# ZhangHH233/Retinal_OCT_Image_Segmentation_via_Deep_Learning

Hardware: AMD Instinct MI355X
Metric: B-scans/sec (train fwd+bwd) at batch 32, 512x1024 (higher is better)
Workload: dtype bf16; 1 GPU; SOTAS/Layers_Segment UNet(1,8,init_features=32) train step, 512x1024, batch 32/GPU (BASELINE configs[1]); global_batch=32, parallelism=dp1, hip_graph=False

## Files before the change

include/oct_hip.h:

```cpp
#ifndef OCT_HIP_H
#define OCT_HIP_H

#include <stddef.h>
#include <stdint.h>

#ifdef __cplusplus
extern "C" {
#endif

#define OCT_VERSION 220

#define OCT_DT_BF16 0
#define OCT_DT_F32 1

#define OCT_OK 0
#define OCT_IMG_SHIFT_ALL 2
#define OCT_E_INVALID (-22)
#define OCT_E_LAUNCH (-5)
#define OCT_E_NODEVICE (-19)

#define OCT_XF_NONE 0
#define OCT_XF_AFFINE_RELU 1
#define OCT_XF_AFFINE 2

// ... 19 lines not shown
int oct_device_count(void);

typedef struct OctConvDesc {
  int dtype;
  int n, h, w;
  int c0, c1;
  int cout;
  int taps;
  int xform0, xform1;
  int in_mode, out_mode;
  int split;
  int want_stats;
  int kh, kw;
  int depth;
  int out_img_mul, out_img_add;
} OctConvDesc;

typedef struct OctConvArgs {
  const void* x0; const void* x1;
  const float* scale0; const float* shift0;
  const float* scale1; const float* shift1;
  const void* wpacked;
  const float* bias;
  void* y0; void* y1;
  float* stat_partials;
} OctConvArgs;

int oct_conv_stat_blocks(const OctConvDesc* d);
size_t oct_packed_weight_elems(int rows, int taps, int kch);
int oct_pack_weights(int mode, int dtype, const float* w, void* wpacked, int cout, int cin, void* stream);
int oct_pack_weights_kk(int mode, int dtype, const float* w, void* wpacked, int cout, int cin, int kh, int kw,
                        void* stream);
int oct_pack_weights3d(int mode, int dtype, const float* w, void* wpacked, int cout, int cin, int kdi, void* stream);
#define OCT_PACK_BATCH_MAX 96
typedef struct OctPackJob {
  int mode, cout, cin, reserved;
  const float* w;
  void* wpacked;
} OctPackJob;
int oct_pack_weights_batch(int dtype, int count, const OctPackJob* jobs, void* stream);
int oct_conv_forward(const OctConvDesc* d, const OctConvArgs* a, void* stream);

typedef struct OctWgradDesc {
  int dtype;
  int n, h, w;
  int c0, c1;
  int cout;
  int taps;
  int xform0, xform1;
  int dy_mode;
  int kh, kw;
  int depth;
  int in_img_shift;
  int dy_img_mul, dy_img_add;
  int partials;
} OctWgradDesc;
typedef struct OctWgradArgs {
  const void* x0; const void* x1;
  const float* scale0; const float* shift0;
  const float* scale1; const float* shift1;
  const void* dy;
  float* dwp;
  float* dbias;
  const void* dy_y; const float* dy_coef; const float* dy_scale; const float* dy_shift;
  float* dbias_partials;
} OctWgradArgs;
int oct_conv_wgrad(const OctWgradDesc* d, const OctWgradArgs* a, void* stream);
int oct_conv_wgrad_partials(const OctWgradDesc* d);
int oct_reduce_bias_partials(const float* part, int nparts, int rows, int channels, float* dbias, int accumulate,
                             void* stream);
int oct_conv_wgrad_fused_apply_ok(const OctWgradDesc* d);
int oct_conv_wgrad_all_depth_taps_ok(const OctWgradDesc* d);
int oct_unpack_wgrad(int mode, const float* dwp, float* grad, int cout, int cin, int accumulate, void* stream);
int oct_unpack_wgrad_kk(const float* dwp, float* grad, int cout, int cin, int kh, int kw, int accumulate, void* stream);
int oct_unpack_wgrad3d(int mode, const float* dwp, float* grad, int cout, int cin, int kdi, int accumulate, void* stream);
typedef struct OctUnpackJob {
  int mode, cout, cin, accumulate;
  int nparts, reserved;
  const float* dwp;
  float* grad;
} OctUnpackJob;
int oct_unpack_wgrad_batch(int count, const OctUnpackJob* jobs, void* stream);

int oct_bn_finalize(const float* partials, int nblocks, int c, double count,
                    const float* gamma, const float* beta, float eps, float momentum,
                    float* running_mean, float* running_var,
                    float* mean, float* invstd, float* scale, float* shift, const float* conv_bias,
                    void* stream);
int oct_bn_eval_coeffs(int c, const float* gamma, const float* beta, const float* running_mean,
                       const float* running_var, float eps, float* scale, float* shift,
                       const float* conv_bias, void* stream);

int oct_bn_relu_pool_fwd(int dtype, const void* y, const float* scale, const float* shift,
                         void* pooled, int n, int h, int w, int c, void* stream);
int oct_bn_relu_fwd(int dtype, const void* y, const float* scale, const float* shift,
                    void* out, size_t npix, int c, void* stream);

int oct_dact_bn_reduce(int dtype, const void* da, const void* dpool, const void* y,
                       const float* scale, const float* shift, const float* mean,
                       const float* invstd, void* g, float* partials, int n, int h, int w, int c,
                       void* stream);
int oct_dact_bn_reduce_blocks(int n, int h, int w, int c, int has_pool);
int oct_bn_bwd_apply_pool_ok(int dtype, int n, int h, int w, int c);
int oct_bn_bwd_apply_pool(int dtype, const void* da, const void* dpool, const void* y, const float* scale,
                          const float* shift, const float* coef, void* dy, int n, int h, int w, int c, void* stream);
int oct_bn_bwd_finalize(const float* partials, int nblocks, int c, double count,
                        const float* gamma, const float* mean, const float* invstd,
                        float* dgamma, float* dbeta, float* coef , int accumulate,
                        void* stream);
int oct_bn_bwd_apply(int dtype, void* g, const void* y, const float* coef, const float* scale,
                     const float* shift, size_t npix, int c, void* stream);
int oct_bn_bwd_apply_to(int dtype, void* dst, const void* g, const void* y, const float* coef, const float* scale,
                        const float* shift, size_t npix, int c, void* stream);
int oct_rowdot_ok(int c, int k);
int oct_rowdot_blocks(size_t npix, int c);
int oct_rowdot_fwd(int dtype, const void* x, const float* w, void* y, float* stats, size_t npix, int c, int k, void* stream);
int oct_rowdot_bwd_data(int dtype, const void* dy, const float* w, void* dx, size_t npix, int c, int k, void* stream);
int oct_rowdot_bwd_weight(int dtype, const void* dy, const void* x, float* dw, float* partials, size_t npix, int c, int k,
                          int accumulate, void* stream);
int oct_rowdot_bwd_weight_bias(int dtype, const void* dy, const void* x, float* dw, float* dbias, float* partials, size_t npix, int c,
                               int k, int accumulate, void* stream);

int oct_channel_sum(int dtype, const void* x, float* out, size_t npix, int c, int accumulate,
                    void* stream);

typedef struct OctHeadDesc {
  int dtype;
  int n, h, w;
  int feat;
  int classes;
} OctHeadDesc;
#define OCT_MAX_CLASSES 16
#define OCT_HEAD_LOSS_SLOTS (2 + 3 * OCT_MAX_CLASSES)
int oct_head_blocks(const OctHeadDesc* d);
int oct_head_forward(const OctHeadDesc* d, const void* y, const float* scale, const float* shift,
                     const float* w , const float* b, const int64_t* target,
                     float* probs, int64_t* argmax, float* logits ,
                     double* loss_partials, void* stream);
int oct_head_loss_finalize(const OctHeadDesc* d, const double* loss_partials, int nblocks,
                           float w_ce, float w_dice, float dice_eps, float* loss_out,
                           float* dice_coef, void* stream);
int oct_head_dlogits(const OctHeadDesc* d, const void* y, const float* scale, const float* shift,
                     const float* w, const float* b, const int64_t* target, const float* dice_coef,
                     float w_ce, const float* dprobs, void* dlogits, void* stream);

int oct_head_backward_fused(const OctHeadDesc* d, const void* y, const float* scale, const float* shift,
                            const float* mean, const float* invstd, const float* w, const float* b,
                            const int64_t* target, const float* dice_coef, float w_ce,
                            const float* dprobs, void* dlogits, void* da, float* partials,
                            float* dbias, float* dweight, double* loss_partials, void* stream);

#define OCT_SEG_NHWC 0
#define OCT_SEG_NCHW 1
int oct_seg_loss_blocks(size_t npix, int classes);
int oct_seg_loss_forward(const OctHeadDesc* d, int layout, const void* logits, const int64_t* target,
                         int64_t* argmax, double* loss_partials, void* stream);
int oct_seg_loss_backward(const OctHeadDesc* d, int layout, const void* logits, const int64_t* target,
                          const float* dice_coef, float w_ce, const float* dloss, void* dlogits,
                          double* loss_partials, void* stream);

int oct_seg_loss_weight_sum(const OctHeadDesc* d, const int64_t* target, const float* class_weight,
                            const float* pixel_weight, int has_ignore, int64_t ignore_index,
                            double* partials, double* wsum, void* stream);
int oct_seg_loss_forward_weighted(const OctHeadDesc* d, int layout, const void* logits,
                                  const int64_t* target, const float* class_weight,
                                  const float* pixel_weight, int has_ignore, int64_t ignore_index,
// ... 93 lines not shown
```

retinal_oct_image_segmentation_via_deep_learning_amd/_lib.py:

```python
from __future__ import annotations

import ctypes as C
import os
import subprocess
import threading

PKG_DIR = os.path.dirname(os.path.abspath(__file__))
LIB_PATH = os.environ.get("OCT_HIP_LIB") or os.path.join(PKG_DIR, "liboct_hip.so")
CSRC_DIR = os.path.join(PKG_DIR, "csrc")

DT_BF16, DT_F32 = 0, 1
XF_NONE, XF_AFFINE_RELU, XF_AFFINE = 0, 1, 2
IN_PLAIN, IN_S2D = 0, 1
IMG_SHIFT_ALL = 2
ACT_NONE, ACT_RELU, ACT_SIGMOID = 0, 1, 2
ACT_PRELU = 3
OUT_PLAIN, OUT_D2S = 0, 1
PACK_CONV_FPROP, PACK_CONV_DGRAD, PACK_DECONV_FPROP, PACK_DECONV_DGRAD, PACK_1X1_DGRAD, PACK_1X1_FPROP = range(6)
PACK_CONV3D_FPROP, PACK_CONV3D_DGRAD, PACK_DECONV3D_FPROP, PACK_DECONV3D_DGRAD = 6, 7, 8, 9
MAX_CLASSES = 16
HEAD_LOSS_SLOTS = 2 + 3 * MAX_CLASSES
SEG_NHWC, SEG_NCHW = 0, 1

c_void_p, c_int, c_size_t, c_float, c_double = C.c_void_p, C.c_int, C.c_size_t, C.c_float, C.c_double


class PackJob(C.Structure):
    _fields_ = [("mode", c_int), ("cout", c_int), ("cin", c_int), ("reserved", c_int), ("w", c_void_p),
                ("wpacked", c_void_p)]


class UnpackJob(C.Structure):
    _fields_ = [("mode", c_int), ("cout", c_int), ("cin", c_int), ("accumulate", c_int), ("nparts", c_int),
                ("reserved", c_int), ("dwp", c_void_p), ("grad", c_void_p)]


PACK_BATCH_MAX = 96


class ConvDesc(C.Structure):
    _fields_ = [(k, c_int) for k in (
        "dtype", "n", "h", "w", "c0", "c1", "cout", "taps", "xform0", "xform1", "in_mode", "out_mode",
        "split", "want_stats", "kh", "kw", "depth", "out_img_mul", "out_img_add")]


class ConvArgs(C.Structure):
    _fields_ = [(k, c_void_p) for k in (
        "x0", "x1", "scale0", "shift0", "scale1", "shift1", "wpacked", "bias", "y0", "y1", "stat_partials")]


class WgradDesc(C.Structure):
    _fields_ = [(k, c_int) for k in (
        "dtype", "n", "h", "w", "c0", "c1", "cout", "taps", "xform0", "xform1", "dy_mode", "kh", "kw", "depth",
        "in_img_shift", "dy_img_mul", "dy_img_add", "partials")]


class WgradArgs(C.Structure):
    _fields_ = [(k, c_void_p) for k in ("x0", "x1", "scale0", "shift0", "scale1", "shift1", "dy", "dwp", "dbias",
                                                "dy_y", "dy_coef", "dy_scale", "dy_shift", "dbias_partials")]


class HeadDesc(C.Structure):
    _fields_ = [(k, c_int) for k in ("dtype", "n", "h", "w", "feat", "classes")]


SIGNATURES = {
    "oct_version_string": (C.c_char_p, []),
    "oct_version": (c_int, []),
    "oct_get_last_error": (c_int, [C.c_char_p, c_size_t]),
    "oct_device_count": (c_int, []),
    "oct_conv_stat_blocks": (c_int, [C.POINTER(ConvDesc)]),
    "oct_packed_weight_elems": (c_size_t, [c_int, c_int, c_int]),
    "oct_pack_weights": (c_int, [c_int, c_int, c_void_p, c_void_p, c_int, c_int, c_void_p]),
    "oct_pack_weights3d": (c_int, [c_int, c_int, c_void_p, c_void_p, c_int, c_int, c_int, c_void_p]),
    "oct_unpack_wgrad3d": (c_int, [c_int, c_void_p, c_void_p, c_int, c_int, c_int, c_int, c_void_p]),
    "oct_depth_pool_fwd": (c_int, [c_int, c_void_p, c_void_p, c_size_t, c_size_t, c_void_p]),
    "oct_depth_pool_bwd": (c_int, [c_int, c_void_p, c_void_p, c_void_p, c_size_t, c_size_t, c_void_p]),
    "oct_pack_weights_kk": (c_int, [c_int, c_int, c_void_p, c_void_p, c_int, c_int, c_int, c_int, c_void_p]),
    "oct_unpack_wgrad_kk": (c_int, [c_void_p, c_void_p, c_int, c_int, c_int, c_int, c_int, c_void_p]),
    "oct_affine_prelu_fwd": (c_int, [c_int, c_void_p, c_void_p, c_void_p, c_void_p, c_void_p, c_size_t, c_int, c_void_p]),
    "oct_affine_prelu_bwd": (c_int, [c_int, c_void_p, c_void_p, c_void_p, c_void_p, c_void_p, c_void_p, c_void_p, c_size_t,
                                     c_int, c_void_p]),
    "oct_maxpool_idx_fwd": (c_int, [c_int, c_void_p, c_void_p, c_void_p, c_int, c_int, c_int, c_int, c_int, c_void_p]),
    "oct_index_scatter": (c_int, [c_int, c_void_p, c_void_p, c_void_p, c_int, c_size_t, c_size_t, c_int, c_void_p]),
    "oct_index_gather": (c_int, [c_int, c_void_p, c_void_p, c_void_p, c_int, c_size_t, c_size_t, c_int, c_void_p]),
    "oct_prelu_bn_fused_ok": (c_int, [c_int, c_int]),
    "oct_dact_bn_reduce_prelu": (c_int, [c_int, c_void_p, c_void_p, c_void_p, c_void_p, c_void_p, c_void_p, c_void_p, c_void_p, c_void_p,
                                         c_int, c_int, c_int, c_int, c_void_p]),
    "oct_bn_bwd_apply_prelu_to": (c_int, [c_int, c_void_p, c_void_p, c_void_p, c_void_p, c_void_p, c_void_p, c_void_p, c_size_t, c_int,
                                          c_void_p]),
    "oct_maxpool_code_fwd": (c_int, [c_int, c_void_p, c_void_p, c_void_p, c_int, c_int, c_int, c_int, c_int, c_void_p]),
    "oct_window_scatter": (c_int, [c_int, c_void_p, c_void_p, c_void_p, c_int, c_int, c_int, c_int, c_int, c_void_p]),
    "oct_window_gather": (c_int, [c_int, c_void_p, c_void_p, c_void_p, c_int, c_int, c_int, c_int, c_int, c_void_p]),
    "oct_pack_weights_batch": (c_int, [c_int, c_int, C.POINTER(PackJob), c_void_p]),
    "oct_conv_forward": (c_int, [C.POINTER(ConvDesc), C.POINTER(ConvArgs), c_void_p]),
    "oct_conv_wgrad": (c_int, [C.POINTER(WgradDesc), C.POINTER(WgradArgs), c_void_p]),
    "oct_conv_wgrad_fused_apply_ok": (c_int, [C.POINTER(WgradDesc)]),
    "oct_conv_wgrad_all_depth_taps_ok": (c_int, [C.POINTER(WgradDesc)]),
    "oct_conv_wgrad_partials": (c_int, [C.POINTER(WgradDesc)]),
    "oct_reduce_bias_partials": (c_int, [c_void_p, c_int, c_int, c_int, c_void_p, c_int, c_void_p]),
    "oct_unpack_wgrad": (c_int, [c_int, c_void_p, c_void_p, c_int, c_int, c_int, c_void_p]),
    "oct_unpack_wgrad_batch": (c_int, [c_int, C.POINTER(UnpackJob), c_void_p]),
    "oct_bn_finalize": (c_int, [c_void_p, c_int, c_int, c_double, c_void_p, c_void_p, c_float, c_float,
                                c_void_p, c_void_p, c_void_p, c_void_p, c_void_p, c_void_p, c_void_p, c_void_p]),
    "oct_bn_eval_coeffs": (c_int, [c_int, c_void_p, c_void_p, c_void_p, c_void_p, c_float, c_void_p, c_void_p,
                                   c_void_p, c_void_p]),
    "oct_bn_relu_pool_fwd": (c_int, [c_int, c_void_p, c_void_p, c_void_p, c_void_p, c_int, c_int, c_int, c_int,
                                     c_void_p]),
    "oct_bn_relu_fwd": (c_int, [c_int, c_void_p, c_void_p, c_void_p, c_void_p, c_size_t, c_int, c_void_p]),
    "oct_dact_bn_reduce": (c_int, [c_int, c_void_p, c_void_p, c_void_p, c_void_p, c_void_p, c_void_p, c_void_p,
                                   c_void_p, c_void_p, c_int, c_int, c_int, c_int, c_void_p]),
    "oct_dact_bn_reduce_blocks": (c_int, [c_int, c_int, c_int, c_int, c_int]),
    "oct_bn_bwd_apply_pool_ok": (c_int, [c_int, c_int, c_int, c_int, c_int]),
    "oct_bn_bwd_apply_pool": (c_int, [c_int, c_void_p, c_void_p, c_void_p, c_void_p, c_void_p, c_void_p, c_void_p,
                                      c_int, c_int, c_int, c_int, c_void_p]),
    "oct_bn_bwd_finalize": (c_int, [c_void_p, c_int, c_int, c_double, c_void_p, c_void_p, c_void_p, c_void_p,
                                    c_void_p, c_void_p, c_int, c_void_p]),
    "oct_bn_bwd_apply": (c_int, [c_int, c_void_p, c_void_p, c_void_p, c_void_p, c_void_p, c_size_t, c_int,
                                 c_void_p]),
    "oct_bn_bwd_apply_to": (c_int, [c_int, c_void_p, c_void_p, c_void_p, c_void_p, c_void_p, c_void_p, c_size_t, c_int,
                                    c_void_p]),
    "oct_channel_sum": (c_int, [c_int, c_void_p, c_void_p, c_size_t, c_int, c_int, c_void_p]),
    "oct_rowdot_ok": (c_int, [c_int, c_int]),
    "oct_rowdot_blocks": (c_int, [c_size_t, c_int]),
    "oct_rowdot_fwd": (c_int, [c_int, c_void_p, c_void_p, c_void_p, c_void_p, c_size_t, c_int, c_int, c_void_p]),
    "oct_rowdot_bwd_data": (c_int, [c_int, c_void_p, c_void_p, c_void_p, c_size_t, c_int, c_int, c_void_p]),
    "oct_rowdot_bwd_weight": (c_int, [c_int, c_void_p, c_void_p, c_void_p, c_void_p, c_size_t, c_int, c_int, c_int, c_void_p]),
    "oct_rowdot_bwd_weight_bias": (c_int, [c_int, c_void_p, c_void_p, c_void_p, c_void_p, c_void_p, c_size_t, c_int, c_int, c_int,
                                           c_void_p]),
    "oct_head_blocks": (c_int, [C.POINTER(HeadDesc)]),
    "oct_head_forward": (c_int, [C.POINTER(HeadDesc), c_void_p, c_void_p, c_void_p, c_void_p, c_void_p, c_void_p,
                                 c_void_p, c_void_p, c_void_p, c_void_p, c_void_p]),
    "oct_head_loss_finalize": (c_int, [C.POINTER(HeadDesc), c_void_p, c_int, c_float, c_float, c_float, c_void_p,
                                       c_void_p, c_void_p]),
    "oct_head_dlogits": (c_int, [C.POINTER(HeadDesc), c_void_p, c_void_p, c_void_p, c_void_p, c_void_p, c_void_p,
                                 c_void_p, c_float, c_void_p, c_void_p, c_void_p]),
    "oct_head_backward_fused": (c_int, [C.POINTER(HeadDesc), c_void_p, c_void_p, c_void_p, c_void_p, c_void_p, c_void_p,
                                        c_void_p, c_void_p, c_void_p, c_float, c_void_p, c_void_p, c_void_p, c_void_p,
                                        c_void_p, c_void_p, c_void_p, c_void_p]),
    "oct_seg_loss_blocks": (c_int, [c_size_t, c_int]),
    "oct_seg_loss_forward": (c_int, [C.POINTER(HeadDesc), c_int, c_void_p, c_void_p, c_void_p, c_void_p, c_void_p]),
    "oct_seg_loss_backward": (c_int, [C.POINTER(HeadDesc), c_int, c_void_p, c_void_p, c_void_p, c_float, c_void_p, c_void_p,
                                      c_void_p, c_void_p]),
    "oct_seg_loss_weight_sum": (c_int, [C.POINTER(HeadDesc), c_void_p, c_void_p, c_void_p, c_int, C.c_int64, c_void_p, c_void_p,
                                        c_void_p]),
    "oct_seg_loss_forward_weighted": (c_int, [C.POINTER(HeadDesc), c_int, c_void_p, c_void_p, c_void_p, c_void_p, c_int,
                                              C.c_int64, c_void_p, c_void_p]),
    "oct_seg_loss_backward_weighted": (c_int, [C.POINTER(HeadDesc), c_int, c_void_p, c_void_p, c_void_p, c_void_p, c_int,
                                               C.c_int64, c_void_p, c_void_p, c_float, c_void_p, c_void_p, c_void_p, c_void_p]),
    "oct_seg_loss_finalize_weighted": (c_int, [C.POINTER(HeadDesc), c_void_p, c_int, c_float, c_float, c_float, c_void_p,
                                               c_void_p, c_void_p, c_void_p]),
    "oct_nchw_to_nhwc": (c_int, [c_int, c_void_p, c_void_p, c_int, c_int, c_int, c_int, c_void_p]),
    "oct_nhwc_to_nchw": (c_int, [c_int, c_void_p, c_void_p, c_int, c_int, c_int, c_int, c_void_p]),
    "oct_sgd_step": (c_int, [c_void_p, c_void_p, c_void_p, c_size_t, c_float, c_float, c_float, c_float, c_int,
                             c_void_p]),
    "oct_adam_step": (c_int, [c_void_p, c_void_p, c_void_p, c_void_p, c_size_t, c_float, c_float, c_float, c_float, c_float,
                              c_int, c_float, c_float, c_float, c_void_p, c_void_p, c_void_p]),
    "oct_sgd_step_scaled": (c_int, [c_void_p, c_void_p, c_void_p, c_size_t, c_float, c_float, c_float, c_float, c_int,
                                    c_void_p, c_void_p, c_void_p]),
    "oct_grad_norm_blocks": (c_int, [c_size_t]),
    "oct_grad_norm": (c_int, [c_void_p, c_size_t, c_float, c_float, c_void_p, c_void_p, c_void_p]),
    "oct_affine_act_fwd": (c_int, [c_int, c_void_p, c_void_p, c_void_p, c_void_p, c_int, c_void_p, c_size_t, c_int,
                                   c_void_p]),
    "oct_affine_res_act_fwd": (c_int, [c_int, c_void_p, c_void_p, c_void_p, c_void_p, c_void_p, c_int, c_void_p, c_size_t,
                                       c_int, c_void_p]),
    "oct_act_bwd": (c_int, [c_int, c_void_p, c_void_p, c_int, c_void_p, c_size_t, c_void_p]),
    "oct_maxpool_fwd": (c_int, [c_int, c_void_p, c_void_p, c_int, c_int, c_int, c_int, c_int, c_void_p]),
    "oct_maxpool_bwd": (c_int, [c_int, c_void_p, c_void_p, c_void_p, c_int, c_int, c_int, c_int, c_int, c_void_p]),
    "oct_bilinear_up_fwd": (c_int, [c_int, c_void_p, c_void_p, c_int, c_int, c_int, c_int, c_int, c_void_p]),
    "oct_bilinear_up_bwd": (c_int, [c_int, c_void_p, c_void_p, c_int, c_int, c_int, c_int, c_int, c_void_p]),
    "oct_bilinear_resize_fwd": (c_int, [c_int, c_void_p, c_void_p, c_int, c_int, c_int, c_int, c_int, c_int, c_void_p]),
    "oct_bilinear_resize_bwd": (c_int, [c_int, c_void_p, c_void_p, c_int, c_int, c_int, c_int, c_int, c_int, c_void_p]),
    "oct_depth_to_space": (c_int, [c_int, c_void_p, c_void_p, c_void_p, c_int, c_int, c_int, c_int, c_int, c_void_p]),
    "oct_space_to_depth": (c_int, [c_int, c_void_p, c_void_p, c_int, c_int, c_int, c_int, c_int, c_void_p]),
    "oct_gate_fwd": (c_int, [c_int, c_void_p, c_void_p, c_void_p, c_size_t, c_int, c_void_p]),
    "oct_gate_bwd": (c_int, [c_int, c_void_p, c_void_p, c_void_p, c_void_p, c_void_p, c_size_t, c_int, c_void_p]),
    "oct_confusion_counts": (c_int, [c_void_p, c_void_p, c_int, c_size_t, c_void_p, c_void_p, c_void_p]),
    "oct_class_confusion_counts": (c_int, [c_void_p, c_void_p, c_int, c_size_t, c_int, c_void_p, c_void_p, c_void_p]),
    "oct_sqdiff_sum": (c_int, [c_void_p, c_void_p, c_int, c_size_t, c_void_p, c_void_p]),
    "oct_column_absdiff_sum": (c_int, [c_void_p, c_void_p, c_int, c_int, c_size_t, c_size_t, c_void_p, c_void_p]),
}

_lib = None
_lock = threading.Lock()
param_generation = [0]
# ... 50 lines not shown
```

retinal_oct_image_segmentation_via_deep_learning_amd/engine.py:

```python
from __future__ import annotations

import ctypes as C
import os
from dataclasses import dataclass, field

import torch

from . import _lib as L

BN_EPS = 1e-5
BN_MOMENTUM = 0.1

@dataclass
class ConvKeys:
    w: str
    bn: str
    b: str | None = None


@dataclass
class BlockSpec:
    name: str
    c1: ConvKeys
    c2: ConvKeys
# ... 163 lines not shown
        hit = self._packed.get((key, mode))
        if hit is not None and hit[0] == ver and hit[2] == wt.data_ptr():
            return hit[1]
        self._pack_plan[(key, mode)] = (cout, cin)
        rows, taps, kch = {
            L.PACK_CONV_FPROP: (cout, 9, cin), L.PACK_CONV_DGRAD: (cin, 9, cout),
            L.PACK_DECONV_FPROP: (4 * cout, 1, cin), L.PACK_DECONV_DGRAD: (cin, 1, 4 * cout),
            L.PACK_1X1_DGRAD: (cin, 1, cout), L.PACK_1X1_FPROP: (cout, 1, cin),
            L.PACK_CONV3D_FPROP: (cout, 9, 3 * cin), L.PACK_CONV3D_DGRAD: (cin, 9, 3 * cout),
            L.PACK_DECONV3D_FPROP: (4 * cout, 1, cin), L.PACK_DECONV3D_DGRAD: (cin, 1, 8 * cout)}[mode]
        elems = L.lib().oct_packed_weight_elems(rows, taps, kch)
        out = hit[1] if hit is not None else torch.empty(elems, dtype=self.tdt, device=wt.device)
        if mode >= L.PACK_CONV3D_FPROP:
            self._pack_plan.pop((key, mode), None)
            L.check(L.lib().oct_pack_weights3d(mode, self.dt, wt.data_ptr(), out.data_ptr(), cout, cin, kdi, _stream()),
                    "oct_pack_weights3d")
        else:
            L.check(L.lib().oct_pack_weights(mode, self.dt, wt.data_ptr(), out.data_ptr(), cout, cin, _stream()),
                    "oct_pack_weights")
        self._packed[(key, mode)] = (ver, out, wt.data_ptr())
        return out

    def _prepack(self, P: dict) -> None:
        jobs, news = [], []
        for (key, mode), (cout, cin) in self._pack_plan.items():
            wt = P.get(key) if isinstance(key, str) else None
            hit = self._packed.get((key, mode))
            if wt is None or hit is None or hit[2] != wt.data_ptr():
                continue
            ver = (wt._version, L.param_generation[0])
            if hit[0] != ver:
                jobs.append(L.PackJob(mode, cout, cin, 0, wt.data_ptr(), hit[1].data_ptr()))
                news.append(((key, mode), (ver, hit[1], hit[2])))
        if jobs:
            arr = (L.PackJob * len(jobs))(*jobs)
            L.check(L.lib().oct_pack_weights_batch(self.dt, len(jobs), arr, _stream()), "oct_pack_weights_batch")
            self._packed.update(news)

    def _conv(self, src: Src, wpacked, cout, taps, n, h, w, y0, *, y1=None, split=0, in_mode=L.IN_PLAIN,
              out_mode=L.OUT_PLAIN, bias=None, stats=None, kh=0, kw=0, depth=0, oimg=(0, 0)):
        d = L.ConvDesc(self.dt, n, h, w, src.c0, src.c1, cout, taps,
                       _xf(src.bn0), _xf(src.bn1),
                       in_mode, out_mode, split, 1 if stats is not None else 0, kh, kw, depth, oimg[0], oimg[1])
        a = L.ConvArgs(L.ptr(src.x0), L.ptr(src.x1),
                       L.ptr(src.bn0.scale) if src.bn0 else None, L.ptr(src.bn0.shift) if src.bn0 else None,
                       L.ptr(src.bn1.scale) if src.bn1 else None, L.ptr(src.bn1.shift) if src.bn1 else None,
                       L.ptr(wpacked), L.ptr(bias), L.ptr(y0), L.ptr(y1), L.ptr(stats))
        ev = self._prof_begin()
        L.check(L.lib().oct_conv_forward(C.byref(d), C.byref(a), _stream()), "oct_conv_forward")
        self._prof_end(ev, "igemm", (taps, src.channels, cout, n, h, w, in_mode, out_mode))

    def _stat_blocks(self, cout, n, h, w, src: Src, taps=9, kh=0, kw=0, depth=0):
        d = L.ConvDesc(self.dt, n, h, w, src.c0, src.c1, cout, taps,
                       _xf(src.bn0), _xf(src.bn1), 0, 0, 0, 1, kh, kw, depth, 0, 0)
        return L.lib().oct_conv_stat_blocks(C.byref(d))

    def _wgrad(self, src: Src, dy, cout, taps, n, h, w, dy_mode=L.IN_PLAIN, dbias=None, fused_apply=None, kh=0, kw=0,
               depth=0, in_shift=0, dy_img=(0, 0), dwp=None, partials_ok=True):
        ktot = src.channels
        parts = 1 if (self.deterministic and partials_ok and dwp is None and depth == 0) else 0
        d = L.WgradDesc(self.dt, n, h, w, src.c0, src.c1, cout, taps,
                        _xf(src.bn0), _xf(src.bn1), dy_mode, kh, kw, depth, in_shift,
                        dy_img[0], dy_img[1], parts)
        bias_parts = None
        if parts:
            nparts = L.lib().oct_conv_wgrad_partials(C.byref(d))
            dwp = torch.empty((nparts, taps, cout, ktot), dtype=torch.float32, device=dy.device)
            dwp._oct_nparts = nparts
            if dbias is not None:
                bias_parts = torch.empty((nparts, cout), dtype=torch.float32, device=dy.device)
        elif dwp is None:
            dwp = self._dwp_take(taps * cout * ktot, dy.device).view(taps, cout, ktot)
        a = L.WgradArgs(L.ptr(src.x0), L.ptr(src.x1),
                        L.ptr(src.bn0.scale) if src.bn0 else None, L.ptr(src.bn0.shift) if src.bn0 else None,
                        L.ptr(src.bn1.scale) if src.bn1 else None, L.ptr(src.bn1.shift) if src.bn1 else None,
                        L.ptr(dy), L.ptr(dwp), L.ptr(dbias), *([L.ptr(t) for t in fused_apply] if fused_apply
                                                                 else [None, None, None, None]), L.ptr(bias_parts))
        ev = self._prof_begin()
        L.check(L.lib().oct_conv_wgrad(C.byref(d), C.byref(a), _stream()), "oct_conv_wgrad")
        self._prof_end(ev, "wgrad", (taps, ktot, cout, n, h, w, dy_mode, 0))
        if bias_parts is not None:
            L.check(L.lib().oct_reduce_bias_partials(bias_parts.data_ptr(), nparts, cout,
                                                     cout // 4 if dy_mode == L.IN_S2D else cout, dbias.data_ptr(), 1,
                                                     _stream()), "oct_reduce_bias_partials")
        return dwp

    def _dwp_take(self, numel: int, dev) -> torch.Tensor:
        if self._arena_on:
            lo = self._arena_off
            self._arena_off = lo + (numel + 63) // 64 * 64
            if self._arena is not None and self._arena_off <= self._arena.numel() and self._arena.device == dev:
                return self._arena[lo:lo + numel]
            self._arena_short = True
        return torch.zeros(numel, dtype=torch.float32, device=dev)

    def _arena_begin(self, dev):
        self._arena_on, self._arena_off, self._arena_short = True, 0, False
        self._unpack_jobs = []
        if self._arena is not None and self._arena.device == dev:
            self._arena.zero_()

    def _flush_unpack(self):
        if self._unpack_jobs:
            arr = (L.UnpackJob * len(self._unpack_jobs))(*[j[0] for j in self._unpack_jobs])
            L.check(L.lib().oct_unpack_wgrad_batch(len(self._unpack_jobs), arr, _stream()), "oct_unpack_wgrad_batch")
            self._unpack_jobs = []

    def _arena_end(self, dev):
        self._flush_unpack()
        if self._arena_short or self._arena is None:
            self._arena = torch.empty(self._arena_off, dtype=torch.float32, device=dev)
        self._arena_on = False

    def _unpack(self, mode, dwp, grad, cout, cin, accumulate):
        job = L.UnpackJob(mode, cout, cin, int(accumulate), getattr(dwp, "_oct_nparts", 1), 0, dwp.data_ptr(), grad.data_ptr())
        if self._arena_on:
            self._unpack_jobs.append((job, dwp, grad))
            return
        arr = (L.UnpackJob * 1)(job)
        L.check(L.lib().oct_unpack_wgrad_batch(1, arr, _stream()), "oct_unpack_wgrad_batch")

    def _conv_bn(self, P, keys: ConvKeys, src: Src, cout, n, h, w, train: bool) -> ConvRec:
        wkey, nk = keys.w, keys.bn
        wt = P[wkey]
        dev = wt.device
        cbias = L.ptr(P[keys.b]) if keys.b else None
        wp = self._pack(wkey, wt, L.PACK_CONV_FPROP, cout, src.channels)
        y = self._act(n, h, w, cout, dev)
        scale = torch.empty(cout, dtype=torch.float32, device=dev)
        shift = torch.empty_like(scale)
        if train:
            nblk = self._stat_blocks(cout, n, h, w, src)
            partials = torch.empty((nblk, 2, cout), dtype=torch.float32, device=dev)
            self._conv(src, wp, cout, 9, n, h, w, y, stats=partials)
            mean = torch.empty_like(scale)
            invstd = torch.empty_like(scale)
            L.check(L.lib().oct_bn_finalize(
                partials.data_ptr(), nblk, cout, float(n * h * w), P[nk + ".weight"].data_ptr(),
                P[nk + ".bias"].data_ptr(), BN_EPS, BN_MOMENTUM, P[nk + ".running_mean"].data_ptr(),
                P[nk + ".running_var"].data_ptr(), mean.data_ptr(), invstd.data_ptr(), scale.data_ptr(),
                shift.data_ptr(), cbias, _stream()), "oct_bn_finalize")
            self._nbt.append(P[nk + ".num_batches_tracked"])
            bn = BNState(scale, shift, mean, invstd)
        else:
            self._conv(src, wp, cout, 9, n, h, w, y)
            L.check(L.lib().oct_bn_eval_coeffs(
                cout, P[nk + ".weight"].data_ptr(), P[nk + ".bias"].data_ptr(),
                P[nk + ".running_mean"].data_ptr(), P[nk + ".running_var"].data_ptr(), BN_EPS,
                scale.data_ptr(), shift.data_ptr(), cbias, _stream()), "oct_bn_eval_coeffs")
            if self._frozen_bwd:
                invstd = torch.rsqrt(P[nk + ".running_var"] + BN_EPS)
                mean = P[nk + ".running_mean"] - P[keys.b] if keys.b else P[nk + ".running_mean"]
                bn = BNState(scale, shift, mean, invstd, frozen=True)
            else:
                bn = BNState(scale, shift)
        return ConvRec(wkey, nk + ".weight", nk + ".bias", keys.b, src, y, bn, cout, n, h, w)

    def _block(self, P, blk: BlockSpec, src, n, h, w, train, ctx):
        r1 = self._conv_bn(P, blk.c1, src, blk.cout, n, h, w, train)
        r2 = self._conv_bn(P, blk.c2, Src(r1.y, blk.cout, r1.bn), blk.cout, n, h, w, train)
        ctx.convs[blk.name] = [r1, r2]
        return r2

    def forward(self, P: dict, x: torch.Tensor, train: bool, target: torch.Tensor | None = None,
                loss_cfg=(1.0, 0.0, 1e-7), want_probs=True, want_argmax=False, want_logits=False, defer_loss=False,
                frozen_bwd=False):
# ... 190 lines not shown
    def _stage_done(self, hook, idx):
        if hook is not None and idx in hook.flush_stages:
            self._flush_unpack()
            hook.stage_done(idx)

    def backward(self, P: dict, ctx: Ctx, G: dict, dprobs: torch.Tensor | None = None, accumulate=False,
                 dlogits: torch.Tensor | None = None, stage_hook=None):
        lib = L.lib()
        sp = self.spec
        self._P, self._ctx = P, ctx
        n, h, w, f, ncls = ctx.n, ctx.h, ctx.w, self.f, self.ncls
        rec = ctx.head_in
        dev = rec.y.device
        self._arena_begin(dev)
        hd = L.HeadDesc(self.dt, n, h, w, f, ncls)
        if dprobs is not None:
            dprobs = dprobs.to(torch.float32).contiguous()
            tgt, dc, w_ce = None, None, 0.0
        elif dlogits is None:
            if ctx.target is None:
                raise RuntimeError("backward without an output gradient needs forward(target=...)")
            tgt, dc, w_ce = ctx.target, ctx.dice_coef, ctx.loss_cfg[0]
        hsrc = Src(rec.y, f, rec.bn)
        head_partials = None
        hw, hb = P[sp.head_w], P[sp.head_b]
        bgrad, wgrad_t = G[sp.head_b], G[sp.head_w]
        fused_dw = False
        dl = None
        if f == 32 and dlogits is None:
            fused_dw = ncls <= 8
            if not accumulate:
                bgrad.zero_()
                if fused_dw:
                    wgrad_t.zero_()
            if not fused_dw:
                dl = self._act(n, h, w, ncls, dev)
            da = self._act(n, h, w, f, dev)
            nb = lib.oct_head_blocks(C.byref(hd))
            head_partials = torch.empty((nb, 2, f), dtype=torch.float32, device=dev)
            L.check(lib.oct_head_backward_fused(
                C.byref(hd), rec.y.data_ptr(), rec.bn.scale.data_ptr(), rec.bn.shift.data_ptr(),
                rec.bn.mean.data_ptr(), rec.bn.invstd.data_ptr(), hw.data_ptr(),
                hb.data_ptr(), L.ptr(tgt), L.ptr(dc), w_ce, L.ptr(dprobs), L.ptr(dl), da.data_ptr(),
                head_partials.data_ptr(), bgrad.data_ptr(), wgrad_t.data_ptr() if fused_dw else None,
                L.ptr(ctx.loss_partials) if dprobs is None else None, _stream()),
                "oct_head_backward_fused")
            if ctx.loss_partials is not None and dprobs is None:
                w_ce_, w_dice_, eps_ = ctx.loss_cfg
                L.check(lib.oct_head_loss_finalize(C.byref(hd), ctx.loss_partials.data_ptr(), ctx.loss_partials.shape[0],
                                                   w_ce_, w_dice_, eps_, ctx.loss.data_ptr(), ctx.dice_coef.data_ptr(),
                                                   _stream()), "oct_head_loss_finalize")
        else:
            dl = self._act(n, h, w, ncls, dev)
            if dlogits is not None:
                dlf = dlogits.to(torch.float32).contiguous()
                L.check(lib.oct_nchw_to_nhwc(self.dt, dlf.data_ptr(), dl.data_ptr(), n, ncls, h, w, _stream()),
                        "oct_nchw_to_nhwc")
            else:
                L.check(lib.oct_head_dlogits(C.byref(hd), rec.y.data_ptr(), rec.bn.scale.data_ptr(),
                                             rec.bn.shift.data_ptr(), hw.data_ptr(), hb.data_ptr(), L.ptr(tgt),
                                             L.ptr(dc), w_ce, L.ptr(dprobs), dl.data_ptr(), _stream()),
                        "oct_head_dlogits")
            L.check(lib.oct_channel_sum(self.dt, dl.data_ptr(), bgrad.data_ptr(), n * h * w, ncls, int(accumulate),
                                        _stream()), "oct_channel_sum")
            wp = self._pack(sp.head_w, hw, L.PACK_1X1_DGRAD, ncls, f)
            da = self._act(n, h, w, f, dev)
            self._conv(Src(dl, ncls), wp, f, 1, n, h, w, da)
        if not fused_dw:
            dwp = self._wgrad(hsrc, dl, ncls, 1, n, h, w)
            self._unpack(L.PACK_1X1_FPROP, dwp, wgrad_t, ncls, f, accumulate)
        nd = len(sp.dec)
        dskip = [None] * nd
        for di in range(nd - 1, -1, -1):
            d0, d1 = self._block_backward(sp.dec[di].name, da, None, G, accumulate,
                                          partials=head_partials if di == nd - 1 else None)
            du, dskip[di] = (d0, d1) if sp.dec_first else (d1, d0)
            wkey, bkey, cout_d = sp.ups[di]
            prev, u = ctx.ups[di]
            cin_d = prev.cout
            hl, wl = prev.h, prev.w
            bgrad = G[bkey]
            if not accumulate:
                bgrad.zero_()
            dwp = self._wgrad(Src(prev.y, cin_d, prev.bn), du, 4 * cout_d, 1, n, hl, wl, dy_mode=L.IN_S2D,
                              dbias=bgrad)
            self._unpack(L.PACK_DECONV_FPROP, dwp, G[wkey], cout_d, cin_d, accumulate)
            wp = self._pack(wkey, P[wkey], L.PACK_DECONV_DGRAD, cout_d, cin_d)
            da = self._act(n, hl, wl, cin_d, dev)
            self._conv(Src(du, cout_d), wp, cin_d, 1, n, hl, wl, da, in_mode=L.IN_S2D)
            if self.debug is not None:
                self.debug["up:" + wkey] = dict(x=prev.y.float().clone(), bn=(prev.bn.scale.clone(), prev.bn.shift.clone()),
                                                u=u.float().clone(), du=du.float().clone(), da=da.float().clone(), bkey=bkey)
            self._stage_done(stage_hook, nd - 1 - di)
        dpool, _ = self._block_backward(sp.enc[-1].name, da, None, G, accumulate)
        self._stage_done(stage_hook, nd)
        for li in range(len(sp.enc) - 2, -1, -1):
            dpool, _ = self._block_backward(sp.enc[li].name, dskip[nd - 1 - li], dpool, G, accumulate,
                                            need_dx=(li != 0))
            if li:
                self._stage_done(stage_hook, nd + len(sp.enc) - 1 - li)
        self._arena_end(dev)
        self._stage_done(stage_hook, nd + len(sp.enc) - 1)
        self._P = self._ctx = None
        return G
```

Measured before the change: 1208 B-scans/s.

## Fuse transposed-conv backward weight grad, bias grad and input grad into one kernel

Adds a HIP kernel that computes the 2x2 stride-2 deconvolution's weight gradient, bias gradient and input gradient in a single pass. Each tile of the upstream gradient and the BN-transformed input is staged once in LDS and reused for both MFMA products. Previously this took a separate wgrad kernel and a dgrad conv, each reading du from HBM. The fused path applies only to cin 64/128 shapes, and the cost is heavy LDS and register use plus atomics in non-deterministic mode.

```diff
diff --git a/include/oct_hip.h b/include/oct_hip.h
--- a/include/oct_hip.h
+++ b/include/oct_hip.h
@@ -125,6 +125,26 @@
 } OctUnpackJob;
 int oct_unpack_wgrad_batch(int count, const OctUnpackJob* jobs, void* stream);
 
+typedef struct OctDeconvBwdDesc {
+  int dtype;
+  int n, h, w;
+  int cin, cout;
+  int xform;
+  int partials;
+} OctDeconvBwdDesc;
+typedef struct OctDeconvBwdArgs {
+  const void* x; const float* scale; const float* shift;
+  const void* du;
+  const void* wpacked;
+  void* dx;
+  float* dwp;
+  float* dbias;
+  float* dbias_partials;
+} OctDeconvBwdArgs;
+int oct_deconv_backward_ok(const OctDeconvBwdDesc* d);
+int oct_deconv_backward_partials(const OctDeconvBwdDesc* d);
+int oct_deconv_backward(const OctDeconvBwdDesc* d, const OctDeconvBwdArgs* a, void* stream);
+
 int oct_bn_finalize(const float* partials, int nblocks, int c, double count,
                     const float* gamma, const float* beta, float eps, float momentum,
                     float* running_mean, float* running_var,
diff --git a/retinal_oct_image_segmentation_via_deep_learning_amd/_lib.py b/retinal_oct_image_segmentation_via_deep_learning_amd/_lib.py
--- a/retinal_oct_image_segmentation_via_deep_learning_amd/_lib.py
+++ b/retinal_oct_image_segmentation_via_deep_learning_amd/_lib.py
@@ -58,6 +58,14 @@
 class WgradArgs(C.Structure):
     _fields_ = [(k, c_void_p) for k in ("x0", "x1", "scale0", "shift0", "scale1", "shift1", "dy", "dwp", "dbias",
                                                 "dy_y", "dy_coef", "dy_scale", "dy_shift", "dbias_partials")]
+
+
+class DeconvBwdDesc(C.Structure):
+    _fields_ = [(k, c_int) for k in ("dtype", "n", "h", "w", "cin", "cout", "xform", "partials")]
+
+
+class DeconvBwdArgs(C.Structure):
+    _fields_ = [(k, c_void_p) for k in ("x", "scale", "shift", "du", "wpacked", "dx", "dwp", "dbias", "dbias_partials")]
 
 
 class HeadDesc(C.Structure):
@@ -101,6 +109,9 @@
     "oct_reduce_bias_partials": (c_int, [c_void_p, c_int, c_int, c_int, c_void_p, c_int, c_void_p]),
     "oct_unpack_wgrad": (c_int, [c_int, c_void_p, c_void_p, c_int, c_int, c_int, c_void_p]),
     "oct_unpack_wgrad_batch": (c_int, [c_int, C.POINTER(UnpackJob), c_void_p]),
+    "oct_deconv_backward_ok": (c_int, [C.POINTER(DeconvBwdDesc)]),
+    "oct_deconv_backward_partials": (c_int, [C.POINTER(DeconvBwdDesc)]),
+    "oct_deconv_backward": (c_int, [C.POINTER(DeconvBwdDesc), C.POINTER(DeconvBwdArgs), c_void_p]),
     "oct_bn_finalize": (c_int, [c_void_p, c_int, c_int, c_double, c_void_p, c_void_p, c_float, c_float,
                                 c_void_p, c_void_p, c_void_p, c_void_p, c_void_p, c_void_p, c_void_p, c_void_p]),
     "oct_bn_eval_coeffs": (c_int, [c_int, c_void_p, c_void_p, c_void_p, c_void_p, c_float, c_void_p, c_void_p,
diff --git a/retinal_oct_image_segmentation_via_deep_learning_amd/csrc/deconv_bwd.hip b/retinal_oct_image_segmentation_via_deep_learning_amd/csrc/deconv_bwd.hip
--- /dev/null
+++ b/retinal_oct_image_segmentation_via_deep_learning_amd/csrc/deconv_bwd.hip
@@ -0,0 +1,339 @@
+#include "common.h"
+#include <stdlib.h>
+
+struct DeconvBwdParams {
+  const bf16_t* x; const float* sc; const float* sh; const bf16_t* du; const bf16_t* wp;
+  bf16_t* dx; float* dwp; float* dbias; float* dbias_part;
+  int n, h, w, xf, part_mode;
+  int tiles_x, tiles_y, ntiles;
+};
+
+typedef unsigned int db_u32x4 __attribute__((ext_vector_type(4)));
+typedef unsigned int db_u32x2 __attribute__((ext_vector_type(2)));
+typedef short db_s16x4 __attribute__((ext_vector_type(4)));
+
+__device__ __forceinline__ unsigned db_pack(float a, float b) {
+  typedef __bf16 bf16x2 __attribute__((ext_vector_type(2)));
+  bf16x2 v;
+  v[0] = (bf16_t)a;
+  v[1] = (bf16_t)b;
+  return __builtin_bit_cast(unsigned, v);
+}
+
+__device__ __forceinline__ bf16x8 db_tr_frag(const unsigned char* first, const unsigned char* second) {
+  typedef __attribute__((address_space(3))) db_s16x4 lds_s16x4;
+  const db_s16x4 a = __builtin_amdgcn_ds_read_tr16_b64_v4i16((lds_s16x4*)(first));
+  const db_s16x4 b = __builtin_amdgcn_ds_read_tr16_b64_v4i16((lds_s16x4*)(second));
+  typedef short s16x8 __attribute__((ext_vector_type(8)));
+  const s16x8 v = {a[0], a[1], a[2], a[3], b[0], b[1], b[2], b[3]};
+  return __builtin_bit_cast(bf16x8, v);
+}
+
+template <int CIN, int COUT, int TH, bool WREG>
+struct DeconvBwdCfg {
+  static constexpr int TPIX = TH * 32;
+  static constexpr int K4 = 4 * COUT;
+  static constexpr int IB = CIN / 32, CB = K4 / 32;
+  static constexpr int BLKB = TPIX * 64 + 64;
+  static constexpr int NK16 = K4 / 16;
+  static constexpr int XS = 0, DUS = IB * BLKB, SXF = DUS + CB * BLKB, OSCR = SXF + 2 * CIN * 4, WL = OSCR + 8 * 32 * 80;
+  static constexpr int LDS = WL + (WREG ? 0 : CIN * K4 * 2);
+};
+
+template <int CIN, int COUT, int TH, bool WREG>
+__global__ void __launch_bounds__(512) deconv_bwd_kernel(const DeconvBwdParams p) {
+  typedef DeconvBwdCfg<CIN, COUT, TH, WREG> C;
+  typedef Mma<bf16_t> M;
+  typedef M::Frag Frag;
+  constexpr int TPIX = C::TPIX, K4 = C::K4, IB = C::IB, CB = C::CB, BLKB = C::BLKB, NK16 = C::NK16;
+  constexpr int GX = CIN / 8, GD = COUT / 8;
+  constexpr int NX = TPIX * GX / 512;
+  constexpr int ND = TPIX * 4 * GD / 512;
+  constexpr int RPD = 64 * GD;
+  constexpr int NDY = RPD >= 512 ? 2 : 1;
+  constexpr int NPB = TPIX / 32;
+  constexpr int WCB = CB / 4, WIB = IB / 2;
+  constexpr int NK = TPIX / 16;
+  static_assert(NPB * IB == 8, "one (tile row, ci block) of dX per wave");
+  static_assert(NX * 512 == TPIX * GX && ND * 512 == TPIX * 4 * GD && (512 % GX) == 0 && (RPD >= 512 ? RPD == 512 : 512 % RPD == 0), "staging map");
+  static_assert(CB % 4 == 0 && IB % 2 == 0, "4 x 2 wave grid over the dW blocks");
+
+  extern __shared__ __attribute__((aligned(16))) unsigned char smem[];
+  unsigned char* const xs = smem + C::XS;
+  unsigned char* const dus = smem + C::DUS;
+  float* const sxf = reinterpret_cast<float*>(smem + C::SXF);
+  const int tid = threadIdx.x, lane = tid & 63;
+  const int wave = __builtin_amdgcn_readfirstlane(tid >> 6);
+  const int r = lane & 31, hh = lane >> 5, g4 = lane >> 4, li = lane & 15;
+
+  const int t0 = blockIdx.x, tstep = gridDim.x;
+  if (t0 >= p.ntiles) return;
+  const int nstage = (p.ntiles - t0 + tstep - 1) / tstep;
+
+  const bool xf = p.xf != 0;
+  const float flo = xf_floor(p.xf);
+  for (int i = tid; i < CIN; i += 512) { sxf[i] = xf ? p.sc[i] : 1.f; sxf[CIN + i] = xf ? p.sh[i] : 0.f; }
+  if constexpr (!WREG) {
+    const db_u32x4* const src = reinterpret_cast<const db_u32x4*>(p.wp);
+    db_u32x4* const dst = reinterpret_cast<db_u32x4*>(smem + C::WL);
+    for (int i = tid; i < CIN * K4 / 8; i += 512) dst[i] = src[i];
+  }
+
+  unsigned gox[NX], lox[NX], god[ND], lod[ND];
+  const int xg = tid % GX;
+#pragma unroll
+  for (int k = 0; k < NX; ++k) {
+    const int pix = (tid + 512 * k) / GX;
+    const int ly = pix >> 5, lx = pix & 31;
+    gox[k] = (unsigned)(ly * p.w + lx) * (unsigned)(CIN * 2) + (unsigned)xg * 16u;
+    lox[k] = (unsigned)((xg >> 2) * BLKB + pix * 64 + (((xg & 3) ^ ((pix >> 2) & 3)) * 16));
+  }
+  const int dg = tid % GD;
+  const int dcol = (tid / GD) & 63;
+  const int ddx = dcol & 1;
+#pragma unroll
+  for (int k = 0; k < ND; ++k) {
+    const int rr = (tid + 512 * k) / RPD;
+    const int ly = rr >> 1, dy = rr & 1;
+    const int pix = ly * 32 + (dcol >> 1);
+    const int k4 = (dy * 2 + ddx) * COUT + dg * 8;
+    god[k] = (unsigned)((2 * ly + dy) * (2 * p.w) + dcol) * (unsigned)(COUT * 2) + (unsigned)dg * 16u;
+    lod[k] = (unsigned)((k4 >> 5) * BLKB + pix * 64 + ((((k4 & 31) >> 3) ^ ((pix >> 2) & 3)) * 16));
+  }
+  const int dy_fix = ((tid / RPD) & 1);
+
+  db_u32x4 Rxs[NX], Rds[ND];
+  auto issue = [&](int s, db_u32x4 (&Rx)[NX], db_u32x4 (&Rd)[ND]) {
+    int t = t0 + s * tstep;
+    const int txi = t % p.tiles_x; t /= p.tiles_x;
+    const int tyi = t % p.tiles_y; const int img = t / p.tiles_y;
+    const size_t origin = ((size_t)img * p.h + tyi * TH) * p.w + txi * 32;
+    const size_t o2 = ((size_t)img * (2 * p.h) + 2 * tyi * TH) * (size_t)(2 * p.w) + 2 * txi * 32;
+    const unsigned char* const xb = reinterpret_cast<const unsigned char*>(p.x + origin * CIN);
+    const unsigned char* const db = reinterpret_cast<const unsigned char*>(p.du + o2 * COUT);
+#pragma unroll
+    for (int k = 0; k < NX; ++k) Rx[k] = *reinterpret_cast<const db_u32x4*>(xb + gox[k]);
+#pragma unroll
+    for (int k = 0; k < ND; ++k) Rd[k] = *reinterpret_cast<const db_u32x4*>(db + god[k]);
+  };
+  float bsum[NDY][8];
+#pragma unroll
+  for (int a = 0; a < NDY; ++a)
+#pragma unroll
+    for (int e = 0; e < 8; ++e) bsum[a][e] = 0.f;
+  auto commit = [&](const db_u32x4 (&Rx)[NX], const db_u32x4 (&Rd)[ND]) {
+    float s[8], b[8];
+    if (xf) {
+      const f32x4 s0 = *reinterpret_cast<const f32x4*>(sxf + xg * 8), s1 = *reinterpret_cast<const f32x4*>(sxf + xg * 8 + 4);
+      const f32x4 b0 = *reinterpret_cast<const f32x4*>(sxf + CIN + xg * 8), b1 = *reinterpret_cast<const f32x4*>(sxf + CIN + xg * 8 + 4);
+#pragma unroll
+      for (int j = 0; j < 4; ++j) { s[j] = s0[j]; s[4 + j] = s1[j]; b[j] = b0[j]; b[4 + j] = b1[j]; }
+    }
+#pragma unroll
+    for (int k = 0; k < NX; ++k) {
+      db_u32x4 v = Rx[k];
+      if (xf) {
+#pragma unroll
+        for (int e = 0; e < 4; ++e) {
+          const float lo = fmaxf(fmaf(__uint_as_float(v[e] << 16), s[2 * e], b[2 * e]), flo);
+          const float hi = fmaxf(fmaf(__uint_as_float(v[e] & 0xffff0000u), s[2 * e + 1], b[2 * e + 1]), flo);
+          v[e] = db_pack(lo, hi);
+        }
+      }
+      *reinterpret_cast<db_u32x4*>(xs + lox[k]) = v;
+    }
+#pragma unroll
+    for (int k = 0; k < ND; ++k) {
+      const db_u32x4 v = Rd[k];
+      *reinterpret_cast<db_u32x4*>(dus + lod[k]) = v;
+      float* const bs = bsum[NDY == 2 ? (k & 1) : 0];
+#pragma unroll
+      for (int e = 0; e < 4; ++e) {
+        bs[2 * e] += __uint_as_float(v[e] << 16);
+        bs[2 * e + 1] += __uint_as_float(v[e] & 0xffff0000u);
+      }
+    }
+  };
+
+  const int cb0 = (wave >> 1) * WCB, ib0 = (wave & 1) * WIB;
+  f32x16 acc[WCB][WIB];
+#pragma unroll
+  for (int j = 0; j < WCB; ++j)
+#pragma unroll
+    for (int i = 0; i < WIB; ++i)
+#pragma unroll
+      for (int e = 0; e < 16; ++e) acc[j][i][e] = 0.f;
+  const int tr_pix = 8 * (g4 >> 1) + (li >> 2), tr_chunk = 2 * (g4 & 1) + ((li & 3) >> 1), tr_in = 8 * (li & 1);
+  const int tr_lo = tr_pix * 64 + ((tr_chunk ^ (2 * (g4 >> 1))) * 16) + tr_in;
+  const int tr_hi = (tr_pix + 4) * 64 + ((tr_chunk ^ (2 * (g4 >> 1) + 1)) * 16) + tr_in;
+
+  const int pb = wave % NPB, cib = wave / NPB;
+  Frag Wf[WREG ? NK16 : 1];
+  if constexpr (WREG) {
+#pragma unroll
+    for (int kk = 0; kk < NK16; ++kk)
+      Wf[kk] = M::load(reinterpret_cast<const unsigned char*>(p.wp) + ((size_t)(cib * NK16 + kk) * 1024 + (size_t)lane * 16));
+  }
+  const unsigned char* const wl = smem + C::WL + cib * NK16 * 1024 + lane * 16;
+  const int xpix = pb * 32 + r;
+  const unsigned char* const xrow = dus + xpix * 64;
+  const int xsw = (xpix >> 2) & 3;
+  unsigned char* const osc = smem + C::OSCR + wave * (32 * 80);
+
+  auto stage = [&](int s, db_u32x4 (&Rx)[NX], db_u32x4 (&Rd)[ND]) {
+    commit(Rx, Rd);
+    issue(min(s + 1, nstage - 1), Rx, Rd);
+    __syncthreads();
+    {
+      Frag af[2][WCB], bf[2][WIB];
+      auto ld = [&](int k, Frag (&a)[WCB], Frag (&b)[WIB]) {
+#pragma unroll
+        for (int j = 0; j < WCB; ++j) { const unsigned char* q = dus + (cb0 + j) * BLKB + k * (16 * 64); a[j] = db_tr_frag(q + tr_lo, q + tr_hi); }
+#pragma unroll
+        for (int i = 0; i < WIB; ++i) { const unsigned char* q = xs + (ib0 + i) * BLKB + k * (16 * 64); b[i] = db_tr_frag(q + tr_lo, q + tr_hi); }
+      };
+      ld(0, af[0], bf[0]);
+#pragma unroll
+      for (int k = 0; k < NK; ++k) {
+        if (k + 1 < NK) ld(k + 1, af[(k + 1) & 1], bf[(k + 1) & 1]);
+#pragma unroll
+        for (int j = 0; j < WCB; ++j)
+#pragma unroll
+          for (int i = 0; i < WIB; ++i) M::mma(acc[j][i], af[k & 1][j], bf[k & 1][i]);
+      }
+    }
+    {
+      f32x16 dacc;
+      Frag xb[2];
+      auto ldx = [&](int kk) { return M::load(xrow + (kk >> 1) * BLKB + ((((kk & 1) * 2 + hh) ^ xsw) * 16)); };
+      xb[0] = ldx(0);
+#pragma unroll
+      for (int kk = 0; kk < NK16; ++kk) {
+        if (kk + 1 < NK16) xb[(kk + 1) & 1] = ldx(kk + 1);
+        const Frag wf = WREG ? Wf[WREG ? kk : 0] : M::load(wl + kk * 1024);
+        if (kk == 0) M::mma0(dacc, wf, xb[0]); else M::mma(dacc, wf, xb[kk & 1]);
+      }
+      int t = t0 + s * tstep;
+      const int txi = t % p.tiles_x; t /= p.tiles_x;
+      const int tyi = t % p.tiles_y; const int img = t / p.tiles_y;
+      const size_t pix0 = ((size_t)img * p.h + tyi * TH + pb) * p.w + txi * 32;
+      unsigned char* const fb = reinterpret_cast<unsigned char*>(p.dx + pix0 * CIN + cib * 32);
+#pragma unroll
+      for (int g = 0; g < 4; ++g) {
+        const db_u32x2 v = {db_pack(dacc[4 * g], dacc[4 * g + 1]), db_pack(dacc[4 * g + 2], dacc[4 * g + 3])};
+        *reinterpret_cast<db_u32x2*>(osc + r * 80 + (8 * g + 4 * hh) * 2) = v;
+      }
+      db_u32x4 tv[2];
+#pragma unroll
+      for (int k = 0; k < 2; ++k) {
+        const int chunk = lane + 64 * k;
+        tv[k] = *reinterpret_cast<const db_u32x4*>(osc + (chunk >> 2) * 80 + (chunk & 3) * 16);
+      }
+#pragma unroll
+      for (int k = 0; k < 2; ++k) {
+        const int chunk = lane + 64 * k;
+        *reinterpret_cast<db_u32x4*>(fb + ((unsigned)(chunk >> 2) * (unsigned)(CIN * 2) + (unsigned)(chunk & 3) * 16u)) = tv[k];
+      }
+    }
+    __syncthreads();
+  };
+  issue(0, Rxs, Rds);
+  __syncthreads();
+  stage(0, Rxs, Rds);
+  for (int s = 1; s < nstage; ++s) stage(s, Rxs, Rds);
+
+  float* const out = p.dwp + (p.part_mode ? (size_t)blockIdx.x * (size_t)(K4 * CIN) : 0);
+#pragma unroll
+  for (int j = 0; j < WCB; ++j)
+#pragma unroll
+    for (int i = 0; i < WIB; ++i) {
+      const int ci = (ib0 + i) * 32 + r;
+#pragma unroll
+      for (int e = 0; e < 16; ++e) {
+        const int co = (cb0 + j) * 32 + (e & 3) + 8 * (e >> 2) + 4 * hh;
+        float* const q = &out[(size_t)co * CIN + ci];
+        if (p.part_mode) *q = acc[j][i][e]; else atomicAdd(q, acc[j][i][e]);
+      }
+    }
+  if (p.dbias != nullptr || p.dbias_part != nullptr) {
+    float* const sb = reinterpret_cast<float*>(smem);
+#pragma unroll
+    for (int a = 0; a < NDY; ++a) {
+      const int dy = NDY == 2 ? a : dy_fix;
+#pragma unroll
+      for (int e = 0; e < 8; ++e) sb[((dy * 2 + ddx) * COUT + dg * 8 + e) * 33 + (dcol >> 1)] = bsum[a][e];
+    }
+    __syncthreads();
+    if (tid < K4) {
+      float v = 0.f;
+      for (int c = 0; c < 32; ++c) v += sb[tid * 33 + c];
+      if (p.part_mode) p.dbias_part[(size_t)blockIdx.x * K4 + tid] = v;
+      else atomicAdd(&p.dbias[tid % COUT], v);
+    }
+  }
+}
+
+static bool deconv_fused_enabled() {
+  static const bool on = [] {
+    const char* v2 = getenv("OCT_DISABLE_V2");
+    const char* e = getenv("OCT_DISABLE_DECONV_FUSED");
+    return !(v2 && v2[0] == '1') && !(e && e[0] == '1');
+  }();
+  return on;
+}
+
+static int deconv_bwd_th(int cin, int cout) {
+  if (cin == 64 && cout == 32) return 4;
+  if (cin == 128 && cout == 64) return 2;
+  return 0;
+}
+
+extern "C" int oct_deconv_backward_ok(const OctDeconvBwdDesc* d) {
+  if (!d || !deconv_fused_enabled()) return 0;
+  if (d->dtype != OCT_DT_BF16 || d->n <= 0 || d->h <= 0 || d->w <= 0 || d->cin <= 0 || d->cout <= 0) return 0;
+  if (d->xform < OCT_XF_NONE || d->xform > OCT_XF_AFFINE) return 0;
+  if ((d->w % 32) != 0 || (d->cout % 32) != 0 || (d->cin != 64 && d->cin != 128)) return 0;
+  if ((size_t)4 * d->cout * d->cin * 4 > (size_t)128 * 1024) return 0;
+  const int th = deconv_bwd_th(d->cin, d->cout);
+  if (th == 0 || (d->h % th) != 0) return 0;
+  if ((size_t)d->n * d->h * d->w >= ((size_t)1 << 29)) return 0;
+  return 1;
+}
+
+extern "C" int oct_deconv_backward_partials(const OctDeconvBwdDesc* d) {
+  if (!oct_deconv_backward_ok(d)) return 0;
+  const int th = deconv_bwd_th(d->cin, d->cout);
+  const long long ntiles = (long long)(d->w / 32) * (d->h / th) * d->n;
+  return (int)(ntiles < 256 ? ntiles : 256);
+}
+
+template <int CIN, int COUT, int TH, bool WREG>
+static int launch_deconv_bwd(DeconvBwdParams& p, int grid, hipStream_t s) {
+  typedef DeconvBwdCfg<CIN, COUT, TH, WREG> C;
+  static_assert(C::K4 * 33 * 4 <= C::SXF, "the bias reduction fits the stage images");
+  if (const int rc = oct_lds_optin(reinterpret_cast<const void*>(&deconv_bwd_kernel<CIN, COUT, TH, WREG>), C::LDS)) return rc;
+  p.tiles_x = p.w / 32; p.tiles_y = p.h / TH; p.ntiles = p.tiles_x * p.tiles_y * p.n;
+  hipLaunchKernelGGL((deconv_bwd_kernel<CIN, COUT, TH, WREG>), dim3(grid), dim3(512), C::LDS, s, p);
+  return OCT_OK;
+}
+
+extern "C" int oct_deconv_backward(const OctDeconvBwdDesc* d, const OctDeconvBwdArgs* a, void* stream) {
+  OCT_CHECK(d && a, "oct_deconv_backward: null descriptor");
+  OCT_CHECK(oct_deconv_backward_ok(d), "oct_deconv_backward: descriptor not accepted (oct_deconv_backward_ok): dtype=%d n=%d h=%d w=%d cin=%d "
+            "cout=%d xform=%d", d->dtype, d->n, d->h, d->w, d->cin, d->cout, d->xform);
+  OCT_CHECK(a->x && a->du && a->wpacked && a->dx && a->dwp, "oct_deconv_backward: null tensor");
+  OCT_CHECK(!(d->xform && (!a->scale || !a->shift)), "oct_deconv_backward: xform without scale/shift");
+  OCT_CHECK(!d->partials || !a->dbias || a->dbias_partials, "oct_deconv_backward: partials mode with a bias gradient needs dbias_partials");
+  DeconvBwdParams p;
+  p.x = (const bf16_t*)a->x; p.sc = a->scale; p.sh = a->shift; p.du = (const bf16_t*)a->du; p.wp = (const bf16_t*)a->wpacked;
+  p.dx = (bf16_t*)a->dx; p.dwp = a->dwp;
+  p.part_mode = d->partials ? 1 : 0;
+  p.dbias = (!p.part_mode) ? a->dbias : nullptr;
+  p.dbias_part = (p.part_mode && a->dbias) ? a->dbias_partials : nullptr;
+  p.n = d->n; p.h = d->h; p.w = d->w; p.xf = d->xform;
+  const int grid = oct_deconv_backward_partials(d);
+  int rc;
+  if (d->cin == 64) rc = launch_deconv_bwd<64, 32, 4, true>(p, grid, as_stream(stream));
+  else rc = launch_deconv_bwd<128, 64, 2, false>(p, grid, as_stream(stream));
+  return rc ? rc : oct_check_launch("deconv_bwd");
+}
diff --git a/retinal_oct_image_segmentation_via_deep_learning_amd/engine.py b/retinal_oct_image_segmentation_via_deep_learning_amd/engine.py
--- a/retinal_oct_image_segmentation_via_deep_learning_amd/engine.py
+++ b/retinal_oct_image_segmentation_via_deep_learning_amd/engine.py
@@ -269,6 +269,30 @@
         if bias_parts is not None:
             L.check(L.lib().oct_reduce_bias_partials(bias_parts.data_ptr(), nparts, cout,
                                                      cout // 4 if dy_mode == L.IN_S2D else cout, dbias.data_ptr(), 1,
+                                                     _stream()), "oct_reduce_bias_partials")
+        return dwp
+
+    def _deconv_backward(self, src: Src, du, wpacked, cout, n, h, w, dx, dbias):
+        cin = src.channels
+        parts = 1 if self.deterministic else 0
+        d = L.DeconvBwdDesc(self.dt, n, h, w, cin, cout, _xf(src.bn0), parts)
+        if src.c1 or not L.lib().oct_deconv_backward_ok(C.byref(d)):
+            return None
+        bias_parts = None
+        if parts:
+            nparts = L.lib().oct_deconv_backward_partials(C.byref(d))
+            dwp = torch.empty((nparts, 1, 4 * cout, cin), dtype=torch.float32, device=du.device)
+            dwp._oct_nparts = nparts
+            bias_parts = torch.empty((nparts, 4 * cout), dtype=torch.float32, device=du.device)
+        else:
+            dwp = self._dwp_take(4 * cout * cin, du.device).view(1, 4 * cout, cin)
+        a = L.DeconvBwdArgs(L.ptr(src.x0), L.ptr(src.bn0.scale) if src.bn0 else None, L.ptr(src.bn0.shift) if src.bn0 else None,
+                            L.ptr(du), L.ptr(wpacked), L.ptr(dx), L.ptr(dwp), L.ptr(dbias), L.ptr(bias_parts))
+        ev = self._prof_begin()
+        L.check(L.lib().oct_deconv_backward(C.byref(d), C.byref(a), _stream()), "oct_deconv_backward")
+        self._prof_end(ev, "deconv_bwd", (1, cin, 4 * cout, n, h, w, L.IN_S2D, 0))
+        if bias_parts is not None:
+            L.check(L.lib().oct_reduce_bias_partials(bias_parts.data_ptr(), nparts, 4 * cout, cout, dbias.data_ptr(), 1,
                                                      _stream()), "oct_reduce_bias_partials")
         return dwp
 
@@ -625,12 +649,14 @@
             bgrad = G[bkey]
             if not accumulate:
                 bgrad.zero_()
-            dwp = self._wgrad(Src(prev.y, cin_d, prev.bn), du, 4 * cout_d, 1, n, hl, wl, dy_mode=L.IN_S2D,
-                              dbias=bgrad)
-            self._unpack(L.PACK_DECONV_FPROP, dwp, G[wkey], cout_d, cin_d, accumulate)
             wp = self._pack(wkey, P[wkey], L.PACK_DECONV_DGRAD, cout_d, cin_d)
             da = self._act(n, hl, wl, cin_d, dev)
-            self._conv(Src(du, cout_d), wp, cin_d, 1, n, hl, wl, da, in_mode=L.IN_S2D)
+            usrc = Src(prev.y, cin_d, prev.bn)
+            dwp = self._deconv_backward(usrc, du, wp, cout_d, n, hl, wl, da, bgrad)
+            if dwp is None:
+                dwp = self._wgrad(usrc, du, 4 * cout_d, 1, n, hl, wl, dy_mode=L.IN_S2D, dbias=bgrad)
+                self._conv(Src(du, cout_d), wp, cin_d, 1, n, hl, wl, da, in_mode=L.IN_S2D)
+            self._unpack(L.PACK_DECONV_FPROP, dwp, G[wkey], cout_d, cin_d, accumulate)
             if self.debug is not None:
                 self.debug["up:" + wkey] = dict(x=prev.y.float().clone(), bn=(prev.bn.scale.clone(), prev.bn.shift.clone()),
                                                 u=u.float().clone(), du=du.float().clone(), da=da.float().clone(), bkey=bkey)
```

Measured after the change: 1225 B-scans/s, median of 6. 1.4% higher.
